# tuannv-github/srsRAN_Project

Hardware: AMD Instinct MI355X
Metric: PDSCH+PUSCH codeblocks/s @ 100 MHz 273-PRB 4x4 MIMO (PDSCH 4 layers, PUSCH 4 layers x 4 rx) (higher is better)
Workload: dtype int8+fp32; 1 GPU; BASELINE metric (PDSCH+PUSCH codeblocks/s @ 100 MHz 273-PRB 4x4 MIMO): full PDSCH+PUSCH slot pipeline, 100 MHz numerology-1 273 PRB, 256QAM R=948/1024; parallelism=single GPU

## Files before the change

srsran_project_amd/csrc/pdsch_encoder.hip:

```cpp
#include <hip/hip_runtime.h>

#include <algorithm>
#include <atomic>
#include <cstdlib>

#include "crc_device.h"
#include "ldpc_codec_args.h"
#include "ldpc_common.h"
#include "ldpc_encode_device.h"
#include "rate_match_device.h"
#include "sch_args.h"

namespace srs_amd {
namespace {

constexpr uint32_t PE_CW_BYTES  = 66 * MAX_LIFTING_SIZE / 8;
constexpr uint32_t PE_ENC_WORDS = enc_bits_lds_words(22, 46, MAX_LIFTING_SIZE);

__device__ __forceinline__ uint32_t pe_out_byte(const uint8_t* s_cw, const rm_geometry& g, const fast_div& divL,
                                                uint32_t off, uint32_t E, uint32_t Kq, uint32_t b)
{
  uint32_t byte = 0;
#pragma unroll
  for (uint32_t k = 0; k < 8; ++k) {
    const uint32_t gbit = 8 * b + k;
    if (gbit < off || gbit >= off + E) {
      continue;
    }
    const uint32_t o = gbit - off;
    uint32_t       i, j;
    if (g.Qm == 6) {
      i = __umulhi(o >> 1, 0xAAAAAAABu) >> 1;
      j = o - 6 * i;
    } else {
      const uint32_t sh = g.Qm == 8 ? 3 : g.Qm == 4 ? 2 : g.Qm == 2 ? 1 : 0;
      i                 = o >> sh;
      j                 = o & (g.Qm - 1);
    }
    uint32_t w = g.rank0 + j * Kq + i;
    if (w >= g.L) {
      w -= g.L;
      if (w >= g.L) {
        divL.div(w, w);
      }
    }
    const uint32_t p = w < g.nof_info ? w : w + g.F;
    byte |= ((s_cw[p >> 3] >> (7 - (p & 7))) & 1u) << (7 - k);
  }
  return byte;
}

struct pe_lds {
  uint32_t T24b[256];
  uint32_t Ttb[256];
  uint32_t lw[PE_ENC_WORDS];
  uint32_t edges[MAX_EDGES];
  __attribute__((aligned(16))) uint8_t s_cw[PE_CW_BYTES + 8];
  uint32_t partial[4];
};

template <int NT>
__device__ __forceinline__ uint32_t pe_xor(uint32_t v, uint32_t* partial)
{
  if constexpr (NT == 64) {
    return crc_wave_xor(v);
  } else {
    return crc_block_xor<NT>(v, partial);
  }
}

template <int NT>
__device__ __forceinline__ void pe_message(const pdsch_fused_args& a, const tb_desc& d, uint32_t r, uint32_t n_data,
                                           uint32_t kz, uint8_t* s_cw, uint32_t j)
{
  const uint8_t* tb  = a.tbs + d.tb_offset;
  const uint32_t ob  = r * d.cb_info_bits;
  const uint32_t nmb = (kz + 7) / 8;
  if ((ob & 7u) == 0) {
    const uintptr_t base  = reinterpret_cast<uintptr_t>(tb) + ob / 8;
    const uint32_t  nfull = n_data / 32;
    for (uint32_t q = j; q < nfull; q += NT) {
      const uintptr_t  addr = base + 4 * q;
      const uint32_t*  p4   = reinterpret_cast<const uint32_t*>(addr & ~uintptr_t(3));
      const uint32_t   sh   = static_cast<uint32_t>(addr & 3u);
      const uint32_t   lo   = p4[0];
      const uint32_t   hi   = sh != 0 ? p4[1] : 0u;
      reinterpret_cast<uint32_t*>(s_cw)[q] = sh != 0 ? __builtin_amdgcn_alignbyte(hi, lo, sh) : lo;
    }
    for (uint32_t q = nfull + j; q < (nmb + 3) / 4; q += NT) {
      uint32_t w = 0;
      for (uint32_t b = 0; b < 4; ++b) {
        const uint32_t jb = 4 * q + b;
        uint32_t       v  = 0;
        for (uint32_t k = 0; k < 8 && 8 * jb + k < n_data; ++k) {
          const uint32_t p = ob + 8 * jb + k;
          v |= ((tb[p >> 3] >> (7 - (p & 7))) & 1u) << (7 - k);
        }
        w |= v << (8 * b);
      }
      reinterpret_cast<uint32_t*>(s_cw)[q] = w;
    }
    return;
  }
  for (uint32_t q = j; q < (nmb + 3) / 4; q += NT) {
    uint32_t w = 0;
#pragma unroll
    for (uint32_t b = 0; b < 4; ++b) {
      const uint32_t jb = 4 * q + b;
      uint32_t       v  = 0;
      if (8 * jb + 8 <= n_data) {
        const uint32_t p  = ob + 8 * jb;
        const uint32_t sh = p & 7u;
        uint32_t       x  = static_cast<uint32_t>(tb[p >> 3]) << 8;
        if (sh != 0) {
          x |= tb[(p >> 3) + 1];
        }
        v = (x >> (8 - sh)) & 0xffu;
      } else if (8 * jb < n_data) {
        for (uint32_t k = 0; k < 8 && 8 * jb + k < n_data; ++k) {
          const uint32_t p = ob + 8 * jb + k;
          v |= ((tb[p >> 3] >> (7 - (p & 7))) & 1u) << (7 - k);
        }
      }
      w |= v << (8 * b);
    }
    reinterpret_cast<uint32_t*>(s_cw)[q] = w;
  }
}

__device__ __forceinline__ void pe_crc24_pair(const uint8_t* s_cw, uint32_t b0, uint32_t b1, uint32_t n,
                                              uint32_t polyA, const uint32_t* tableA, const uint32_t* TA,
                                              uint32_t polyB, const uint32_t* tableB, const uint32_t* TB,
                                              uint32_t& outA, uint32_t& outB)
{
  outA = 0;
  outB = 0;
  if (b0 >= b1) {
    return;
  }
  constexpr uint32_t highbit = 1u << 24, mask = highbit - 1u;
  const uint32_t     full    = min(b1, n / 8);
  uint32_t           rA = 0, rB = 0;
  for (uint32_t b = b0; b < full; b += CRC_FETCH_BATCH) {
    uint32_t v[CRC_FETCH_BATCH];
#pragma unroll
    for (uint32_t k = 0; k < CRC_FETCH_BATCH; ++k) {
      v[k] = b + k < full ? s_cw[b + k] : 0u;
    }
#pragma unroll
    for (uint32_t k = 0; k < CRC_FETCH_BATCH; ++k) {
      if (b + k < full) {
        rA = TA[rA >> 16] ^ ((rA << 8) & mask) ^ v[k];
        rB = TB[rB >> 16] ^ ((rB << 8) & mask) ^ v[k];
      }
    }
  }
  for (uint32_t b = max(b0, full); b < b1; ++b) {
    const uint32_t byte = s_cw[b];
    const int      nb   = (b * 8 + 8 <= n) ? 8 : static_cast<int>(n - b * 8);
    for (int i = 0; i < nb; ++i) {
      const uint32_t bit = (byte >> (7 - i)) & 1u;
      rA                 = (rA << 1) | bit;
      rB                 = (rB << 1) | bit;
      rA ^= (rA & highbit) ? polyA : 0u;
      rB ^= (rB & highbit) ? polyB : 0u;
    }
  }
  const uint32_t  e  = min(n, b1 * 8);
  const uint32_t* ta = tableA + (n - e);
  const uint32_t* tb = tableB + (n - e);
#pragma unroll
  for (uint32_t j = 0; j < 24; ++j) {
    outA ^= ta[j] & (0u - ((rA >> j) & 1u));
    outB ^= tb[j] & (0u - ((rB >> j) & 1u));
  }
}

template <int NT>
__device__ __forceinline__ void pe_finish(const pdsch_fused_args& a, pe_lds& s, uint32_t cb, uint32_t t,
                                          const tb_desc& d, uint32_t j, uint32_t& staged_off, uint32_t& staged_ne)
{
  const rm_geometry  g   = a.geos[a.row_geo[cb]];
  const enc_row_desc er  = a.enc_rows[cb];
  const uint32_t     E   = a.row_E[cb];
  const uint32_t     off = a.row_out[cb];
  const uint32_t     Z   = er.Z;
  const uint32_t     Kb  = g.nof_sys / Z + 2;
  const int          bg  = Kb == 22 ? 1 : 2;
  const uint32_t     kz  = Kb * Z;
  uint8_t*           s_cw = s.s_cw;
  if (d.nof_segments > 1) {
    const uint32_t cbi = d.cb_info_bits;
    const uint32_t nb  = (cbi + 7) / 8;
    const uint32_t per = (nb + NT - 1) / NT;
    const uint32_t b0  = j * per;
    const uint32_t r   = cb - d.row0;
    uint32_t       crc;
    if (r + 1 < d.nof_segments) {
      uint32_t tb_part;
      pe_crc24_pair(s_cw, b0, min(nb, b0 + per), cbi, a.crc24b_poly, a.crc24b_table, s.T24b, a.crc24a_poly,
                    a.crc24a_table, s.Ttb, crc, tb_part);
      crc     = pe_xor<NT>(crc, s.partial);
      tb_part = pe_xor<NT>(tb_part, s.partial);
      if (j == 0) {
        a.tb_parts[static_cast<size_t>(t) * a.part_stride + r] = tb_part;
      }
    } else {
      crc = pe_xor<NT>(crc_chunk_contrib(lds_chunk_fetch{s_cw, 0}, b0, min(nb, b0 + per), cbi, 24, a.crc24b_poly,
                                         a.crc24b_table, s.T24b),
                       s.partial);
    }
    if (j == 0) {
      attach_crc_bits(s_cw, cbi, 24, crc);
    }
    __syncthreads();
  }
  const uint32_t nq  = (Z + 31) / 32;
  const uint32_t ncw = enc_bits_cw_words(Kb, er.M_eff, Z);
  uint32_t*      cwb = s.lw;
  uint32_t*      lam = s.lw + ncw;
  uint32_t*      ls  = lam + 4 * nq;
  const uint32_t nmw = (kz + 31) / 32;
  for (uint32_t w = j; w < ncw; w += NT) {
    uint32_t v = 0;
    if (w < nmw) {
      v = __builtin_bitreverse32(__builtin_bswap32(reinterpret_cast<const uint32_t*>(s_cw)[w]));
      if (32 * w + 32 > kz) {
        v &= (1u << (kz - 32 * w)) - 1u;
      }
    }
    cwb[w] = v;
  }
  for (uint32_t w = j; w < nq + 2; w += NT) {
    ls[w] = 0;
  }
  const uint32_t* ge = a.edges + er.edge_off;
  const uint32_t  ne = static_cast<uint32_t>(a.row_start[bg - 1][er.M_eff]);
  if (er.edge_off != staged_off || ne != staged_ne) {
    for (uint32_t e = j; e < ne; e += NT) {
      s.edges[e] = ge[e];
    }
    staged_off = er.edge_off;
    staged_ne  = ne;
  }
  __syncthreads();
  const int32_t core_a[3] = {static_cast<int32_t>(er.core_a[0]), static_cast<int32_t>(er.core_a[1]),
                             static_cast<int32_t>(er.core_a[2])};
  encode_bits_parity<NT>(cwb, lam, ls, s.edges, a.row_start[bg - 1], bg, Kb, Z, er.M_eff,
                                 static_cast<int32_t>(er.p0_shift), core_a, j);
  const uint32_t nbits = er.pack_bits;
  for (uint32_t m = j; m < (nbits + 31) / 32; m += NT) {
    uint32_t v = lds_bits32(cwb, 2 * Z + 32 * m);
    if (32 * m + 32 > nbits) {
      v &= (1u << (nbits - 32 * m)) - 1u;
    }
    reinterpret_cast<uint32_t*>(s_cw)[m] = __builtin_bswap32(__builtin_bitreverse32(v));
  }
  __syncthreads();
  const fast_div divL(g.L);
  const uint32_t Kq    = E / g.Qm;
  const uint32_t first = (off + 7) / 8;
  const uint32_t whole = (off + E) / 8;
  const uint32_t G        = ((off & 7u) == 0 && g.Qm >= 2) ? Kq / 8 : 0;
  const uint32_t fast_end = first + G * g.Qm;
  for (uint32_t gi = j; gi < G; gi += NT) {
    uint64_t x = 0;
#pragma unroll
    for (uint32_t jj = 0; jj < 8; ++jj) {
      if (jj < g.Qm) {
        uint32_t w = g.rank0 + jj * Kq + 8 * gi;
        if (w >= g.L) {
          w -= g.L;
          if (w >= g.L) {
            divL.div(w, w);
          }
        }
        x |= static_cast<uint64_t>(rm_walk_byte(s_cw, g, w)) << (56 - 8 * jj);
      }
    }
    x            = transpose8x8(x);
    uint64_t acc = 0;
#pragma unroll
    for (uint32_t q = 0; q < 8; ++q) {
      acc = (acc << g.Qm) | ((x >> (64 - 8 * q - g.Qm)) & ((1u << g.Qm) - 1u));
    }
    uint8_t* o = a.cw + first + gi * g.Qm;
    for (uint32_t q = 0; q < g.Qm; ++q) {
      o[q] = static_cast<uint8_t>(acc >> (8 * (g.Qm - 1 - q)));
    }
  }
  for (uint32_t b = fast_end + j; b < whole; b += NT) {
    a.cw[b] = static_cast<uint8_t>(pe_out_byte(s_cw, g, divL, off, E, Kq, b));
  }
  if (j < 2) {
    const bool     last_seg = cb == d.row0 + d.nof_segments - 1;
    const uint32_t b        = j == 0 ? off / 8 : whole;
    const bool partial =
        j == 0 ? (off & 7u) != 0 : ((off + E) & 7u) != 0 && (whole != off / 8 || (off & 7u) == 0);
    if (partial) {
      uint32_t mask = 0;
      for (uint32_t k = 0; k < 8; ++k) {
        const uint32_t gbit = 8 * b + k;
        mask |= (gbit >= off && (gbit < off + E || last_seg)) ? (0x80u >> k) : 0u;
      }
      const uint32_t v  = pe_out_byte(s_cw, g, divL, off, E, Kq, b);
      uint32_t*      w4 = reinterpret_cast<uint32_t*>(a.cw + (b & ~3u));
      const uint32_t sh = 8 * (b & 3u);
      atomicAnd(w4, ~(mask << sh));
      atomicOr(w4, v << sh);
    }
  }
  __syncthreads();
}

template <int NT>
__global__ __launch_bounds__(NT) void pdsch_cb_kernel(pdsch_fused_args a)
{
  __shared__ pe_lds s;
  crc_table8_init<NT>(s.T24b, 24, a.crc24b_poly);
  crc_table8_init<NT>(s.Ttb, 24, a.crc24a_poly);
  uint32_t       tb_table_order = 24;
  uint32_t       staged_off = 0, staged_ne = 0;
  const uint32_t j              = threadIdx.x;

  const uint32_t n = a.last_only == 1 ? a.nof_tbs : a.nof_cbs;
  for (uint32_t k = blockIdx.x; k < n; k += gridDim.x) {
    const uint32_t cb   = a.last_only == 1 ? a.last_rows[k] : k;
    const uint32_t t    = a.row_tb[cb];
    const tb_desc  d    = a.tds[t];
    const uint32_t r    = cb - d.row0;
    const uint32_t C    = d.nof_segments;
    const bool     last = r == C - 1;
    if ((a.last_only == 0) == last) {
      continue;
    }
    const uint32_t L    = d.tb_crc_bits;
    const uint32_t n_data = last ? d.cb_info_bits - L - d.zero_pad : d.cb_info_bits;
    const uint32_t kz     = (a.geos[a.row_geo[cb]].nof_sys / a.enc_rows[cb].Z + 2) * a.enc_rows[cb].Z;
    uint32_t tb_crc = 0;
    if (last) {
      if (tb_table_order != L) {
        crc_table8_init<NT>(s.Ttb, L, L == 16 ? a.crc16_poly : a.crc24a_poly);
        tb_table_order = L;
      }
      for (uint32_t i = j; i + 1 < C; i += NT) {
        tb_crc ^= crc_move(a.tb_parts[static_cast<size_t>(t) * a.part_stride + i],
                           d.tbs_bits - (i + 1) * d.cb_info_bits, 24, a.crc24a_table);
      }
    }
    pe_message<NT>(a, d, r, n_data, kz, s.s_cw, j);
    __syncthreads();
    if (last) {
      const uint32_t nb  = (n_data + 7) / 8;
      const uint32_t per = (nb + NT - 1) / NT;
      const uint32_t b0  = j * per;
      tb_crc ^= crc_chunk_contrib(lds_chunk_fetch{s.s_cw, 0}, b0, min(nb, b0 + per), n_data, L,
                                  L == 16 ? a.crc16_poly : a.crc24a_poly, L == 16 ? a.crc16_table : a.crc24a_table,
                                  s.Ttb);
      tb_crc = pe_xor<NT>(tb_crc, s.partial);
      if (j == 0) {
        attach_crc_bits(s.s_cw, n_data, L, tb_crc);
      }
      __syncthreads();
    }
    pe_finish<NT>(a, s, cb, t, d, j, staged_off, staged_ne);
  }
}

constexpr int PE_MAX_DEVICES = 64;

template <int NT>
uint32_t pe_resident_workgroups()
{
  static std::atomic<uint32_t> known[PE_MAX_DEVICES] = {};
  int                          dev = 0, per_cu = 0, cus = 0;
  if (hipGetDevice(&dev) != hipSuccess || dev < 0 || dev >= PE_MAX_DEVICES) {
    (void)hipGetLastError();
    return 65535u;
  }
  uint32_t n = known[dev].load(std::memory_order_relaxed);
  if (n == 0) {
    if (hipDeviceGetAttribute(&cus, hipDeviceAttributeMultiprocessorCount, dev) != hipSuccess || cus <= 0 ||
        hipOccupancyMaxActiveBlocksPerMultiprocessor(&per_cu, pdsch_cb_kernel<NT>, NT, 0) != hipSuccess ||
        per_cu <= 0) {
      (void)hipGetLastError();
      return 65535u;
    }
    n = static_cast<uint32_t>(per_cu) * static_cast<uint32_t>(cus);
    known[dev].store(n, std::memory_order_relaxed);
  }
  return n;
}

}

hipError_t launch_pdsch_fused(const pdsch_fused_args& a, hipStream_t stream)
{
  if (a.nof_cbs == 0) {
    return hipSuccess;
  }
  const char* wg       = std::getenv("SRSRAN_AMD_PDSCH_WG");
  const char* tail     = std::getenv("SRSRAN_AMD_PDSCH_TAIL_WG");
  const bool  big      = wg != nullptr && wg[0] == '2';
  const bool  big_tail = tail == nullptr || tail[0] == '2';
  const char*    gs  = std::getenv("SRSRAN_AMD_PDSCH_GRID");
  const uint32_t cap = gs != nullptr && std::atoi(gs) > 0 ? static_cast<uint32_t>(std::atoi(gs))
                       : big                              ? pe_resident_workgroups<256>()
                                                          : pe_resident_workgroups<64>();
  auto cb_launch = [&](uint32_t last_only, uint32_t n, bool wide) {
    pdsch_fused_args x = a;
    x.last_only        = last_only;
    const dim3 grid(std::min(n, last_only == 0 ? std::min(cap, 65535u) : 65535u));
    if (wide) {
      hipLaunchKernelGGL(pdsch_cb_kernel<256>, grid, dim3(256), 0, stream, x);
    } else {
      hipLaunchKernelGGL(pdsch_cb_kernel<64>, grid, dim3(64), 0, stream, x);
    }
  };
  if (a.nof_cbs > a.nof_tbs) {
    cb_launch(0, a.nof_cbs, big);
  }
  cb_launch(1, a.nof_tbs, big_tail);
  return hipGetLastError();
}

}
```

srsran_project_amd/csrc/rate_match_device.h:

```cpp
#pragma once

#include <hip/hip_runtime.h>

#include "rate_matching_common.h"
#include <cstdint>

namespace srs_amd {

struct fast_div {
  uint32_t d;
  float    rcp;
  __device__ explicit fast_div(uint32_t d_) : d(d_), rcp(1.0f / static_cast<float>(d_ ? d_ : 1)) {}
  __device__ __forceinline__ uint32_t div(uint32_t n, uint32_t& r) const
  {
    uint32_t q = static_cast<uint32_t>(static_cast<float>(n) * rcp);
    int32_t  x = static_cast<int32_t>(n - q * d);
    if (x < 0) {
      q -= 1;
      x += static_cast<int32_t>(d);
    } else if (x >= static_cast<int32_t>(d)) {
      q += 1;
      x -= static_cast<int32_t>(d);
    }
    r = static_cast<uint32_t>(x);
    return q;
  }
};

__device__ __forceinline__ uint64_t transpose8x8(uint64_t x)
{
  uint64_t t = (x ^ (x >> 7)) & 0x00AA00AA00AA00AAull;
  x          = x ^ t ^ (t << 7);
  t          = (x ^ (x >> 14)) & 0x0000CCCC0000CCCCull;
  x          = x ^ t ^ (t << 14);
  t          = (x ^ (x >> 28)) & 0x00000000F0F0F0F0ull;
  return x ^ t ^ (t << 28);
}

__device__ __forceinline__ uint32_t rm_walk_byte(const uint8_t* s_cw, const rm_geometry& g, uint32_t w)
{
  if (w + 7 < g.L && (w + 7 < g.nof_info || w >= g.nof_info)) {
    const uint32_t p = w < g.nof_info ? w : w + g.F;
    const uint32_t v = (static_cast<uint32_t>(s_cw[p >> 3]) << 8) | s_cw[(p >> 3) + 1];
    return (v >> (8 - (p & 7))) & 0xffu;
  }
  uint32_t row = 0;
#pragma unroll
  for (uint32_t k = 0; k < 8; ++k) {
    uint32_t ww = w + k;
    ww          = ww >= g.L ? ww - g.L : ww;
    const uint32_t p = ww < g.nof_info ? ww : ww + g.F;
    row |= ((s_cw[p >> 3] >> (7 - (p & 7))) & 1u) << (7 - k);
  }
  return row;
}

}
```

Baseline: 25.81 million codeblocks/s.

## Rate-match PDSCH codeblocks directly from encoder LDS words with 32-bit walks

Adds a fast path for byte-aligned segments with modest circular-buffer wraparound. It reads encoded bits straight from the encoder's LDS word buffer 32 bits at a time, interleaves them with 8x8 bit transposes and writes the output as 32-bit or 128-bit stores. This skips the repack pass into the byte codeword buffer, the barrier after it, and the per-byte walk and byte stores. It also adds optional timestamp probes that compile out by default. The trade-off is more complex interleaving code and higher register use, with edge bytes still handled bit by bit.

```diff
diff --git a/srsran_project_amd/csrc/pdsch_encoder.hip b/srsran_project_amd/csrc/pdsch_encoder.hip
--- a/srsran_project_amd/csrc/pdsch_encoder.hip
+++ b/srsran_project_amd/csrc/pdsch_encoder.hip
@@ -14,10 +14,40 @@
 namespace srs_amd {
 namespace {
 
+#ifdef SRS_AMD_PDSCH_PROBE
+constexpr uint32_t PE_PROBE_WG = 8192;
+__device__ uint64_t g_pdsch_probe[2][PE_PROBE_WG][16];
+#define PE_STAMP(k, i)                                                                                               \
+  do {                                                                                                               \
+    if (threadIdx.x == 0 && blockIdx.x < PE_PROBE_WG) {                                                              \
+      g_pdsch_probe[k][blockIdx.x][i] =                                                                              \
+          (i) == 0 || (i) == 15 ? __builtin_amdgcn_s_memrealtime() : __builtin_amdgcn_s_memtime();                   \
+    }                                                                                                                \
+  } while (0)
+#else
+#define PE_STAMP(k, i)                                                                                               \
+  do {                                                                                                               \
+  } while (0)
+#endif
+
 constexpr uint32_t PE_CW_BYTES  = 66 * MAX_LIFTING_SIZE / 8;
 constexpr uint32_t PE_ENC_WORDS = enc_bits_lds_words(22, 46, MAX_LIFTING_SIZE);
 
-__device__ __forceinline__ uint32_t pe_out_byte(const uint8_t* s_cw, const rm_geometry& g, const fast_div& divL,
+struct pe_byte_bits {
+  const uint8_t* s_cw;
+  __device__ __forceinline__ uint32_t operator()(uint32_t p) const { return (s_cw[p >> 3] >> (7 - (p & 7))) & 1u; }
+};
+struct pe_word_bits {
+  const uint32_t* cwb;
+  uint32_t        base;
+  __device__ __forceinline__ uint32_t operator()(uint32_t p) const
+  {
+    return (cwb[(base + p) >> 5] >> ((base + p) & 31u)) & 1u;
+  }
+};
+
+template <typename Bits>
+__device__ __forceinline__ uint32_t pe_out_byte(const Bits& bit, const rm_geometry& g, const fast_div& divL,
                                                 uint32_t off, uint32_t E, uint32_t Kq, uint32_t b)
 {
   uint32_t byte = 0;
@@ -45,9 +75,85 @@
       }
     }
     const uint32_t p = w < g.nof_info ? w : w + g.F;
-    byte |= ((s_cw[p >> 3] >> (7 - (p & 7))) & 1u) << (7 - k);
+    byte |= bit(p) << (7 - k);
   }
   return byte;
+}
+
+template <int NT, typename Bits>
+__device__ __forceinline__ void pe_edge_bytes(const Bits& bit, uint8_t* cw, const rm_geometry& g, const fast_div& divL,
+                                              uint32_t off, uint32_t E, uint32_t Kq, uint32_t from, bool last_seg,
+                                              uint32_t j)
+{
+  const uint32_t whole = (off + E) / 8;
+  for (uint32_t b = from + j; b < whole; b += NT) {
+    cw[b] = static_cast<uint8_t>(pe_out_byte(bit, g, divL, off, E, Kq, b));
+  }
+  if (j < 2) {
+    const uint32_t b = j == 0 ? off / 8 : whole;
+    const bool partial =
+        j == 0 ? (off & 7u) != 0 : ((off + E) & 7u) != 0 && (whole != off / 8 || (off & 7u) == 0);
+    if (partial) {
+      uint32_t mask = 0;
+      for (uint32_t k = 0; k < 8; ++k) {
+        const uint32_t gbit = 8 * b + k;
+        mask |= (gbit >= off && (gbit < off + E || last_seg)) ? (0x80u >> k) : 0u;
+      }
+      const uint32_t v  = pe_out_byte(bit, g, divL, off, E, Kq, b);
+      uint32_t*      w4 = reinterpret_cast<uint32_t*>(cw + (b & ~3u));
+      const uint32_t sh = 8 * (b & 3u);
+      atomicAnd(w4, ~(mask << sh));
+      atomicOr(w4, v << sh);
+    }
+  }
+}
+
+template <int NT, uint32_t QM>
+__device__ __forceinline__ void pe_rm_words(const uint32_t* cwb, uint32_t base, uint8_t* seg, const rm_geometry& g,
+                                            uint32_t E, uint32_t Kq, uint32_t j)
+{
+  typedef uint32_t u32x4 __attribute__((ext_vector_type(4), aligned(4)));
+  const uint32_t nd      = E / 32;
+  const bool     aligned = (reinterpret_cast<uintptr_t>(seg) & 3u) == 0;
+  for (uint32_t d0 = QM * j; d0 < nd; d0 += QM * NT) {
+    const uint32_t i0 = 32 * (d0 / QM);
+    uint32_t       row[QM], out[QM];
+#pragma unroll
+    for (uint32_t jj = 0; jj < QM; ++jj) {
+      uint32_t w = g.rank0 + jj * Kq + i0;
+      w -= w >= g.L ? g.L : 0u;
+      row[jj] = rm_walk32(cwb, base, g, w);
+    }
+    rm_interleave32<QM>(row, out);
+    uint8_t* o = seg + 4 * d0;
+    if (aligned && d0 + QM <= nd) {
+      if constexpr (QM % 4 == 0) {
+#pragma unroll
+        for (uint32_t q = 0; q < QM; q += 4) {
+          *reinterpret_cast<u32x4*>(o + 4 * q) = u32x4{out[q], out[q + 1], out[q + 2], out[q + 3]};
+        }
+      } else {
+#pragma unroll
+        for (uint32_t q = 0; q < QM; ++q) {
+          reinterpret_cast<uint32_t*>(o)[q] = out[q];
+        }
+      }
+    } else {
+#pragma unroll
+      for (uint32_t q = 0; q < QM; ++q) {
+        if (d0 + q < nd) {
+          if (aligned) {
+            reinterpret_cast<uint32_t*>(o)[q] = out[q];
+          } else {
+#pragma unroll
+            for (uint32_t b = 0; b < 4; ++b) {
+              o[4 * q + b] = static_cast<uint8_t>(out[q] >> (8 * b));
+            }
+          }
+        }
+      }
+    }
+  }
 }
 
 struct pe_lds {
@@ -215,6 +321,7 @@
     }
     __syncthreads();
   }
+  PE_STAMP(a.last_only, 3);
   const uint32_t nq  = (Z + 31) / 32;
   const uint32_t ncw = enc_bits_cw_words(Kb, er.M_eff, Z);
   uint32_t*      cwb = s.lw;
@@ -244,73 +351,76 @@
     staged_ne  = ne;
   }
   __syncthreads();
+  PE_STAMP(a.last_only, 4);
   const int32_t core_a[3] = {static_cast<int32_t>(er.core_a[0]), static_cast<int32_t>(er.core_a[1]),
                              static_cast<int32_t>(er.core_a[2])};
   encode_bits_parity<NT>(cwb, lam, ls, s.edges, a.row_start[bg - 1], bg, Kb, Z, er.M_eff,
                                  static_cast<int32_t>(er.p0_shift), core_a, j);
-  const uint32_t nbits = er.pack_bits;
-  for (uint32_t m = j; m < (nbits + 31) / 32; m += NT) {
-    uint32_t v = lds_bits32(cwb, 2 * Z + 32 * m);
-    if (32 * m + 32 > nbits) {
-      v &= (1u << (nbits - 32 * m)) - 1u;
-    }
-    reinterpret_cast<uint32_t*>(s_cw)[m] = __builtin_bswap32(__builtin_bitreverse32(v));
+  PE_STAMP(a.last_only, 5);
+  const fast_div divL(g.L);
+  const uint32_t Kq       = E / g.Qm;
+  const uint32_t first    = (off + 7) / 8;
+  const bool     last_seg = cb == d.row0 + d.nof_segments - 1;
+  if (g.Qm >= 2 && (off & 7u) == 0 && g.L >= 32 && g.rank0 + E <= 2 * g.L) {
+    PE_STAMP(a.last_only, 6);
+    uint8_t* seg = a.cw + first;
+    switch (g.Qm) {
+      case 2:
+        pe_rm_words<NT, 2>(cwb, 2 * Z, seg, g, E, Kq, j);
+        break;
+      case 4:
+        pe_rm_words<NT, 4>(cwb, 2 * Z, seg, g, E, Kq, j);
+        break;
+      case 6:
+        pe_rm_words<NT, 6>(cwb, 2 * Z, seg, g, E, Kq, j);
+        break;
+      default:
+        pe_rm_words<NT, 8>(cwb, 2 * Z, seg, g, E, Kq, j);
+        break;
+    }
+    pe_edge_bytes<NT>(pe_word_bits{cwb, 2 * Z}, a.cw, g, divL, off, E, Kq, first + E / 32 * 4, last_seg, j);
+  } else {
+    const uint32_t nbits = er.pack_bits;
+    for (uint32_t m = j; m < (nbits + 31) / 32; m += NT) {
+      uint32_t v = lds_bits32(cwb, 2 * Z + 32 * m);
+      if (32 * m + 32 > nbits) {
+        v &= (1u << (nbits - 32 * m)) - 1u;
+      }
+      reinterpret_cast<uint32_t*>(s_cw)[m] = __builtin_bswap32(__builtin_bitreverse32(v));
+    }
+    __syncthreads();
+    PE_STAMP(a.last_only, 6);
+    const uint32_t G = ((off & 7u) == 0 && g.Qm >= 2) ? Kq / 8 : 0;
+    for (uint32_t gi = j; gi < G; gi += NT) {
+      uint64_t x = 0;
+#pragma unroll
+      for (uint32_t jj = 0; jj < 8; ++jj) {
+        if (jj < g.Qm) {
+          uint32_t w = g.rank0 + jj * Kq + 8 * gi;
+          if (w >= g.L) {
+            w -= g.L;
+            if (w >= g.L) {
+              divL.div(w, w);
+            }
+          }
+          x |= static_cast<uint64_t>(rm_walk_byte(s_cw, g, w)) << (56 - 8 * jj);
+        }
+      }
+      x            = transpose8x8(x);
+      uint64_t acc = 0;
+#pragma unroll
+      for (uint32_t q = 0; q < 8; ++q) {
+        acc = (acc << g.Qm) | ((x >> (64 - 8 * q - g.Qm)) & ((1u << g.Qm) - 1u));
+      }
+      uint8_t* o = a.cw + first + gi * g.Qm;
+      for (uint32_t q = 0; q < g.Qm; ++q) {
+        o[q] = static_cast<uint8_t>(acc >> (8 * (g.Qm - 1 - q)));
+      }
+    }
+    pe_edge_bytes<NT>(pe_byte_bits{s_cw}, a.cw, g, divL, off, E, Kq, first + G * g.Qm, last_seg, j);
   }
   __syncthreads();
-  const fast_div divL(g.L);
-  const uint32_t Kq    = E / g.Qm;
-  const uint32_t first = (off + 7) / 8;
-  const uint32_t whole = (off + E) / 8;
-  const uint32_t G        = ((off & 7u) == 0 && g.Qm >= 2) ? Kq / 8 : 0;
-  const uint32_t fast_end = first + G * g.Qm;
-  for (uint32_t gi = j; gi < G; gi += NT) {
-    uint64_t x = 0;
-#pragma unroll
-    for (uint32_t jj = 0; jj < 8; ++jj) {
-      if (jj < g.Qm) {
-        uint32_t w = g.rank0 + jj * Kq + 8 * gi;
-        if (w >= g.L) {
-          w -= g.L;
-          if (w >= g.L) {
-            divL.div(w, w);
-          }
-        }
-        x |= static_cast<uint64_t>(rm_walk_byte(s_cw, g, w)) << (56 - 8 * jj);
-      }
-    }
-    x            = transpose8x8(x);
-    uint64_t acc = 0;
-#pragma unroll
-    for (uint32_t q = 0; q < 8; ++q) {
-      acc = (acc << g.Qm) | ((x >> (64 - 8 * q - g.Qm)) & ((1u << g.Qm) - 1u));
-    }
-    uint8_t* o = a.cw + first + gi * g.Qm;
-    for (uint32_t q = 0; q < g.Qm; ++q) {
-      o[q] = static_cast<uint8_t>(acc >> (8 * (g.Qm - 1 - q)));
-    }
-  }
-  for (uint32_t b = fast_end + j; b < whole; b += NT) {
-    a.cw[b] = static_cast<uint8_t>(pe_out_byte(s_cw, g, divL, off, E, Kq, b));
-  }
-  if (j < 2) {
-    const bool     last_seg = cb == d.row0 + d.nof_segments - 1;
-    const uint32_t b        = j == 0 ? off / 8 : whole;
-    const bool partial =
-        j == 0 ? (off & 7u) != 0 : ((off + E) & 7u) != 0 && (whole != off / 8 || (off & 7u) == 0);
-    if (partial) {
-      uint32_t mask = 0;
-      for (uint32_t k = 0; k < 8; ++k) {
-        const uint32_t gbit = 8 * b + k;
-        mask |= (gbit >= off && (gbit < off + E || last_seg)) ? (0x80u >> k) : 0u;
-      }
-      const uint32_t v  = pe_out_byte(s_cw, g, divL, off, E, Kq, b);
-      uint32_t*      w4 = reinterpret_cast<uint32_t*>(a.cw + (b & ~3u));
-      const uint32_t sh = 8 * (b & 3u);
-      atomicAnd(w4, ~(mask << sh));
-      atomicOr(w4, v << sh);
-    }
-  }
-  __syncthreads();
+  PE_STAMP(a.last_only, 7);
 }
 
 template <int NT>
@@ -322,6 +432,8 @@
   uint32_t       tb_table_order = 24;
   uint32_t       staged_off = 0, staged_ne = 0;
   const uint32_t j              = threadIdx.x;
+  PE_STAMP(a.last_only, 0);
+  PE_STAMP(a.last_only, 8);
 
   const uint32_t n = a.last_only == 1 ? a.nof_tbs : a.nof_cbs;
   for (uint32_t k = blockIdx.x; k < n; k += gridDim.x) {
@@ -335,6 +447,7 @@
       continue;
     }
     const uint32_t L    = d.tb_crc_bits;
+    PE_STAMP(a.last_only, 1);
     const uint32_t n_data = last ? d.cb_info_bits - L - d.zero_pad : d.cb_info_bits;
     const uint32_t kz     = (a.geos[a.row_geo[cb]].nof_sys / a.enc_rows[cb].Z + 2) * a.enc_rows[cb].Z;
     uint32_t tb_crc = 0;
@@ -363,8 +476,11 @@
       }
       __syncthreads();
     }
+    PE_STAMP(a.last_only, 2);
     pe_finish<NT>(a, s, cb, t, d, j, staged_off, staged_ne);
   }
+  PE_STAMP(a.last_only, 9);
+  PE_STAMP(a.last_only, 15);
 }
 
 constexpr int PE_MAX_DEVICES = 64;
@@ -425,3 +541,23 @@
 }
 
 }
+
+#ifdef SRS_AMD_PDSCH_PROBE
+extern "C" int srs_amd_pdsch_probe_read(void* host, uint64_t bytes, int clear)
+{
+  using namespace srs_amd;
+  if (bytes > sizeof(g_pdsch_probe)) {
+    bytes = sizeof(g_pdsch_probe);
+  }
+  if (hipMemcpyFromSymbol(host, HIP_SYMBOL(g_pdsch_probe), bytes) != hipSuccess) {
+    return -1;
+  }
+  if (clear) {
+    static const uint64_t zero[2 * PE_PROBE_WG * 16] = {};
+    if (hipMemcpyToSymbol(HIP_SYMBOL(g_pdsch_probe), zero, sizeof(zero)) != hipSuccess) {
+      return -2;
+    }
+  }
+  return 0;
+}
+#endif
diff --git a/srsran_project_amd/csrc/rate_match_device.h b/srsran_project_amd/csrc/rate_match_device.h
--- a/srsran_project_amd/csrc/rate_match_device.h
+++ b/srsran_project_amd/csrc/rate_match_device.h
@@ -2,6 +2,7 @@
 
 #include <hip/hip_runtime.h>
 
+#include "ldpc_encode_device.h"
 #include "rate_matching_common.h"
 #include <cstdint>
 
@@ -55,4 +56,81 @@
   return row;
 }
 
+
+__device__ __forceinline__ uint32_t rm_walk_linear32(const uint32_t* cwb, uint32_t base, const rm_geometry& g,
+                                                     uint32_t w)
+{
+  if (w >= g.nof_info) {
+    return lds_bits32(cwb, base + w + g.F);
+  }
+  uint32_t v = lds_bits32(cwb, base + w);
+  if (w + 32 > g.nof_info) {
+    const uint32_t n1 = g.nof_info - w;
+    v                 = (v & ((1u << n1) - 1u)) | (lds_bits32(cwb, base + g.nof_sys) << n1);
+  }
+  return v;
 }
+
+__device__ __forceinline__ uint32_t rm_walk32(const uint32_t* cwb, uint32_t base, const rm_geometry& g, uint32_t w)
+{
+  uint32_t v = rm_walk_linear32(cwb, base, g, w);
+  if (w + 32 > g.L) {
+    const uint32_t n1 = g.L - w;
+    v                 = (v & ((1u << n1) - 1u)) | (rm_walk_linear32(cwb, base, g, 0) << n1);
+  }
+  return v;
+}
+
+template <uint32_t QM>
+__device__ __forceinline__ void rm_interleave32(const uint32_t (&row)[QM], uint32_t (&out)[QM])
+{
+  static_assert(QM == 2 || QM == 4 || QM == 6 || QM == 8, "modulation order");
+  uint32_t r8[8], o8[8] = {};
+#pragma unroll
+  for (uint32_t j = 0; j < 8; ++j) {
+    r8[j] = j < QM ? row[j % QM] : 0u;
+  }
+  uint64_t acc[4] = {};
+#pragma unroll
+  for (uint32_t c = 0; c < 4; ++c) {
+    uint32_t hi = 0, lo = 0;
+#pragma unroll
+    for (uint32_t j = 0; j < 4; ++j) {
+      hi |= ((r8[j] >> (8 * c)) & 0xffu) << (24 - 8 * j);
+      lo |= ((r8[j + 4] >> (8 * c)) & 0xffu) << (24 - 8 * j);
+    }
+    const uint64_t x = transpose8x8((static_cast<uint64_t>(hi) << 32) | lo);
+    if (QM == 8) {
+      o8[2 * c]     = static_cast<uint32_t>(x);
+      o8[2 * c + 1] = static_cast<uint32_t>(x >> 32);
+    } else {
+#pragma unroll
+      for (uint32_t b = 0; b < 8; ++b) {
+        acc[c] |= ((x >> (8 * b + 8 - QM)) & ((1u << QM) - 1u)) << (QM * (7 - b));
+      }
+    }
+  }
+  if (QM == 4) {
+#pragma unroll
+    for (uint32_t c = 0; c < 4; ++c) {
+      o8[c] = __builtin_bswap32(static_cast<uint32_t>(acc[c]));
+    }
+  } else if (QM == 2) {
+    o8[0] = __builtin_bswap32(static_cast<uint32_t>(acc[0] << 16 | acc[1]));
+    o8[1] = __builtin_bswap32(static_cast<uint32_t>(acc[2] << 16 | acc[3]));
+  } else if (QM == 6) {
+#pragma unroll
+    for (uint32_t h = 0; h < 2; ++h) {
+      const uint64_t a = acc[2 * h], b = acc[2 * h + 1];
+      o8[3 * h]     = __builtin_bswap32(static_cast<uint32_t>(a >> 16));
+      o8[3 * h + 1] = __builtin_bswap32(static_cast<uint32_t>(a << 16) | static_cast<uint32_t>(b >> 32));
+      o8[3 * h + 2] = __builtin_bswap32(static_cast<uint32_t>(b));
+    }
+  }
+#pragma unroll
+  for (uint32_t j = 0; j < QM; ++j) {
+    out[j] = o8[j];
+  }
+}
+
+}
```

New measurement: 25.76 million codeblocks/s. About the same (-0.2%).
